# zhaoruiyang98/eftpipe

Hardware: AMD Instinct MI355X
Metric: theory P_l(k) evaluations/sec (single tracer, Nk=512, l=0,2,4) (higher is better)
Workload: dtype f64

## Files before the change

### eftpipe_amd/csrc/eftb_kernels.hpp

```cpp
#pragma once
#include <hip/hip_runtime.h>
#include <stdint.h>

namespace eftb {

constexpr int NS = 80;
constexpr int NPOW = 257;
constexpr int NHALF = 128;
constexpr int NCH = 129;

constexpr int NROW = 24;

typedef double v4d __attribute__((ext_vector_type(4)));
typedef double v2d __attribute__((ext_vector_type(2)));

__device__ __forceinline__ void xcd_decode(int ntile, int& tile, int& group) {
    const int flat = blockIdx.x, ng = gridDim.x / ntile;
    if ((ng & 7) == 0) {
        const int slot = flat >> 3;
        tile = slot % ntile;
        group = (flat & 7) + 8 * (slot / ntile);
    } else {
        tile = flat % ntile;
        group = flat / ntile;
    }
}

template <bool LO>
__device__ __forceinline__ void prep_rows_body(int Nkin, int ntail, int nxtail, int KP1, int KP2, int KP3, int Bmax,
                                                        const double* __restrict__ Pin, const double* __restrict__ lnkin,
                                                        const double* __restrict__ lnxtail, const double* __restrict__ lnxxtail,
                                                        const double* __restrict__ wq2, double* __restrict__ A1, double* __restrict__ A2,
                                                        double* __restrict__ A2T, double* __restrict__ A3, int* __restrict__ status,
                                                        int ntail_lo, int nxtail_lo) {
    extern __shared__ double sm[];
    double* pin = sm;
    const int w = blockIdx.x, tid = threadIdx.x;
    bool bad = false;
    for (int j = tid; j < Nkin; j += blockDim.x) {
        const double v = Pin[(size_t)w * Nkin + j];
        pin[j] = v;
        bad = bad || !(fabs(v) <= 1.79769313486231570815e308) || (j >= Nkin - 2 && !(v > 0.0));
        if (LO) bad = bad || (j < 2 && !(v > 0.0));
    }
    if (bad && status) atomicMax(status, w + 1);
    __syncthreads();
    const double dln = lnkin[Nkin - 1] - lnkin[Nkin - 2];
    const double dlo = LO ? lnkin[1] - lnkin[0] : 0.0;
    if (A1) {
        const double slope = (log(pin[Nkin - 1]) - log(pin[Nkin - 2])) / dln;
        const double amp = pin[Nkin - 1] * exp(-slope * lnkin[Nkin - 1]);
        double slo = 0.0, alo = 0.0;
        if (LO && ntail_lo) {
            slo = (log(pin[1]) - log(pin[0])) / dlo;
            alo = pin[0] * exp(-slo * lnkin[0]);
        }
        const int nhi = ntail - (LO ? ntail_lo : 0);
        for (int j = tid; j < KP1; j += blockDim.x) A1[(size_t)w * KP1 + j] = j < Nkin ? pin[j] : 0.0;
        for (int j = tid; j < KP2; j += blockDim.x) {
            double v = j < Nkin ? pin[j] : (j < Nkin + ntail ? amp * exp(slope * lnxtail[j - Nkin]) : 0.0);
            if (LO && j >= Nkin + nhi && j < Nkin + ntail) v = alo * exp(slo * lnxtail[j - Nkin]);
            A2[(size_t)w * KP2 + j] = v;
            A2T[(size_t)j * Bmax + w] = v;
        }
    }
    if (A3) {
        const double q1 = pin[Nkin - 1] * wq2[1], q0 = pin[Nkin - 2] * wq2[0];
        const double slope = (log(q1) - log(q0)) / dln;
        const double amp = q1 * exp(-slope * lnkin[Nkin - 1]);
        double slo = 0.0, alo = 0.0;
        if (LO && nxtail_lo) {
            const double p0 = pin[0] * wq2[2], p1 = pin[1] * wq2[3];
            slo = (log(p1) - log(p0)) / dlo;
            alo = p0 * exp(-slo * lnkin[0]);
        }
        const int nhi = nxtail - (LO ? nxtail_lo : 0);
        for (int j = tid; j < KP3; j += blockDim.x) {
            double v = j < Nkin ? pin[j] : (j < Nkin + nxtail ? amp * exp(slope * lnxxtail[j - Nkin]) : 0.0);
            if (LO && j >= Nkin + nhi && j < Nkin + nxtail) v = alo * exp(slo * lnxxtail[j - Nkin]);
            A3[(size_t)w * KP3 + j] = v;
        }
    }
}

#define PREP_ROWS_PARAMS int Nkin, int ntail, int nxtail, int KP1, int KP2, int KP3, int Bmax, const double* __restrict__ Pin, \
    const double* __restrict__ lnkin, const double* __restrict__ lnxtail, const double* __restrict__ lnxxtail, const double* __restrict__ wq2, \
    double* __restrict__ A1, double* __restrict__ A2, double* __restrict__ A2T, double* __restrict__ A3, int* __restrict__ status
#define PREP_ROWS_ARGS Nkin, ntail, nxtail, KP1, KP2, KP3, Bmax, Pin, lnkin, lnxtail, lnxxtail, wq2, A1, A2, A2T, A3, status

__global__ __launch_bounds__(256) void prep_rows_kernel(PREP_ROWS_PARAMS) {
    prep_rows_body<false>(PREP_ROWS_ARGS, 0, 0);
}

__global__ __launch_bounds__(256) void prep_rows_lo_kernel(PREP_ROWS_PARAMS, int ntail_lo, int nxtail_lo) {
    prep_rows_body<true>(PREP_ROWS_ARGS, ntail_lo, nxtail_lo);
}

__device__ __forceinline__ void qf_body(int w, int nq, const double* __restrict__ fgrow, const double* __restrict__ Qpoly, double* __restrict__ Q) {
    const int tid = threadIdx.x;
    const double f = fgrow[w];
    for (int idx = tid; idx < 2 * nq; idx += blockDim.x) {
        const int a = idx / nq, rest = idx % nq;
        const double* c = Qpoly + ((size_t)(1 - a) * nq + rest) * 15;
        double cv[15];
#pragma unroll
        for (int p = 0; p < 15; ++p) cv[p] = c[p];
        const double f2 = f * f;
        double ev = cv[14], od = cv[13];
#pragma unroll
        for (int p = 12; p >= 0; p -= 2) {
            ev = fma(ev, f2, cv[p]);
            if (p >= 1) od = fma(od, f2, cv[p - 1]);
        }
        Q[(size_t)w * 2 * nq + idx] = fma(od, f, ev);
    }
}

__global__ __launch_bounds__(256) void prep_rows_qf_kernel(int B, PREP_ROWS_PARAMS, int nq, const double* __restrict__ fgrow,
                                                           const double* __restrict__ Qpoly, double* __restrict__ Q) {
    if ((int)blockIdx.x >= B) {
        qf_body(blockIdx.x - B, nq, fgrow, Qpoly, Q);
        return;
    }
    prep_rows_body<false>(PREP_ROWS_ARGS, 0, 0);
}

__global__ __launch_bounds__(256) void prep_rows_qf_lo_kernel(int B, PREP_ROWS_PARAMS, int nq, const double* __restrict__ fgrow,
                                                              const double* __restrict__ Qpoly, double* __restrict__ Q, int ntail_lo, int nxtail_lo) {
    if ((int)blockIdx.x >= B) {
        qf_body(blockIdx.x - B, nq, fgrow, Qpoly, Q);
        return;
    }
    prep_rows_body<true>(PREP_ROWS_ARGS, ntail_lo, nxtail_lo);
}
#undef PREP_ROWS_PARAMS
#undef PREP_ROWS_ARGS

constexpr int AD_T = NHALF + 2;
constexpr int AD_CH = 1;
constexpr int KSYN = 528;
constexpr int KLIN = 288;
constexpr int SYN_KPAD = 48;
constexpr int SYN_KC = 24;
static_assert(SYN_KPAD % SYN_KC == 0 && (32 * SYN_KC) % 256 == 0, "chunk must divide the padding and fill the staging threads");
constexpr int BAS22 = 8, BASC = 32;

__device__ __forceinline__ double readlane_f64(double v, int lane) {
    return __hiloint2double(__builtin_amdgcn_readlane(__double2hiint(v), lane), __builtin_amdgcn_readlane(__double2loint(v), lane));
}

template <int NC, int NW>
__global__ __launch_bounds__(64 * NW) void antidiag_kernel(int B, int Bmax, const double* __restrict__ coefT,
                                                           const double2* __restrict__ AD, double2* __restrict__ S) {
    constexpr int PB = 3, WPP = 2 * NC;
    static_assert(PB * WPP <= 64, "one wave-load must hold a block's weights");
    __shared__ double red[NW - 1][2 * NC][64];
    const int grp = blockIdx.y, jp = (grp & 1) ? NPOW - 1 - (int)blockIdx.x : (int)blockIdx.x;
    const int lane = threadIdx.x & 63, wave = threadIdx.x >> 6, w = grp * 64 + lane;
    const int wl = w < B ? w : B - 1;
    const int cnt = ((2 * NHALF + jp) >> 1) - jp + 1;
    const int per = (cnt + NW - 1) / NW, t0 = wave * per, t1 = min(cnt, t0 + per);
    const double* cr = coefT + wl;
    const double* ci = coefT + (size_t)NCH * Bmax + wl;
    double ar[NC], ai[NC];
#pragma unroll
    for (int q = 0; q < NC; ++q) ar[q] = ai[q] = 0.0;
    if (t0 < t1) {
        const double* adw = reinterpret_cast<const double*>(AD + ((size_t)jp * AD_T + t0) * NC);
        const int nw = (t1 - t0) * WPP;
        auto wload = [&](int blk) { return adw[min(blk * PB * WPP + lane, nw - 1)]; };
        double xr[PB], xi[PB], yr[PB], yi[PB];
        auto coef = [&](int t, int p) {
            const int n = jp + t, qn = n <= NHALF ? n : 2 * NHALF - n;
            xr[p] = cr[(size_t)qn * Bmax];
            xi[p] = ci[(size_t)qn * Bmax];
            yr[p] = cr[(size_t)t * Bmax];
            yi[p] = ci[(size_t)t * Bmax];
        };
        double wc = wload(0);
#pragma unroll
        for (int p = 0; p < PB; ++p) coef(min(t0 + p, t1 - 1), p);
        const int nblk = (t1 - t0 + PB - 1) / PB;
        for (int blk = 0; blk < nblk; ++blk) {
            const double wn = wload(blk + 1);
#pragma unroll
            for (int p = 0; p < PB; ++p) {
                const int t = t0 + blk * PB + p;
                const double on = t < t1 ? 1.0 : 0.0;
                const double xim = jp + t <= NHALF ? xi[p] : -xi[p], yim = -yi[p];
                const double pr = (xr[p] * yr[p] - xim * yim) * on, pi = (xr[p] * yim + xim * yr[p]) * on;
                __builtin_amdgcn_sched_barrier(0);
                coef(min(t + PB, t1 - 1), p);
                __builtin_amdgcn_sched_barrier(0);
#pragma unroll
                for (int q = 0; q < NC; ++q) {
                    const double mx = readlane_f64(wc, p * WPP + 2 * q), my = readlane_f64(wc, p * WPP + 2 * q + 1);
                    ar[q] = fma(mx, pr, fma(-my, pi, ar[q]));
                    ai[q] = fma(mx, pi, fma(my, pr, ai[q]));
                }
                __builtin_amdgcn_sched_barrier(0);
            }
            wc = wn;
        }
    }
    if (wave > 0) {
#pragma unroll
        for (int q = 0; q < NC; ++q) {
            red[wave - 1][2 * q][lane] = ar[q];
            red[wave - 1][2 * q + 1][lane] = ai[q];
        }
    }
    __syncthreads();
    if (wave == 0 && w < B) {
#pragma unroll
        for (int q = 0; q < NC; ++q) {
#pragma unroll
            for (int v = 0; v < NW - 1; ++v) {
                ar[q] += red[v][2 * q][lane];
                ai[q] += red[v][2 * q + 1][lane];
            }
            S[((size_t)w * NC + q) * NPOW + jp] = make_double2(ar[q], ai[q]);
        }
    }
}

template <int NC, int NW>
__global__ __launch_bounds__(64 * NW) void antidiag_nh_kernel(int B, int Bmax, const double* __restrict__ coefT,
                                                              const double2* __restrict__ AD, double2* __restrict__ S, int nh) {
    constexpr int PB = 3, WPP = 2 * NC;
    static_assert(PB * WPP <= 64, "one wave-load must hold a block's weights");
    __shared__ double red[NW - 1][2 * NC][64];
    const int npow = 2 * nh + 1, nch = nh + 1, adt = nh + 2;
    const int grp = blockIdx.y, jp = (grp & 1) ? npow - 1 - (int)blockIdx.x : (int)blockIdx.x;
    const int lane = threadIdx.x & 63, wave = threadIdx.x >> 6, w = grp * 64 + lane;
    const int wl = w < B ? w : B - 1;
    const int cnt = ((2 * nh + jp) >> 1) - jp + 1;
    const int per = (cnt + NW - 1) / NW, t0 = wave * per, t1 = min(cnt, t0 + per);
    const double* cr = coefT + wl;
    const double* ci = coefT + (size_t)nch * Bmax + wl;
    double ar[NC], ai[NC];
#pragma unroll
    for (int q = 0; q < NC; ++q) ar[q] = ai[q] = 0.0;
    if (t0 < t1) {
        const double* adw = reinterpret_cast<const double*>(AD + ((size_t)jp * adt + t0) * NC);
        const int nw = (t1 - t0) * WPP;
        auto wload = [&](int blk) { return adw[min(blk * PB * WPP + lane, nw - 1)]; };
        double xr[PB], xi[PB], yr[PB], yi[PB];
        auto coef = [&](int t, int p) {
            const int n = jp + t, qn = n <= nh ? n : 2 * nh - n;
            xr[p] = cr[(size_t)qn * Bmax];
            xi[p] = ci[(size_t)qn * Bmax];
            yr[p] = cr[(size_t)t * Bmax];
            yi[p] = ci[(size_t)t * Bmax];
        };
        double wc = wload(0);
#pragma unroll
        for (int p = 0; p < PB; ++p) coef(min(t0 + p, t1 - 1), p);
        const int nblk = (t1 - t0 + PB - 1) / PB;
        for (int blk = 0; blk < nblk; ++blk) {
            const double wn = wload(blk + 1);
#pragma unroll
            for (int p = 0; p < PB; ++p) {
                const int t = t0 + blk * PB + p;
                const double on = t < t1 ? 1.0 : 0.0;
                const double xim = jp + t <= nh ? xi[p] : -xi[p], yim = -yi[p];
                const double pr = (xr[p] * yr[p] - xim * yim) * on, pi = (xr[p] * yim + xim * yr[p]) * on;
                __builtin_amdgcn_sched_barrier(0);
                coef(min(t + PB, t1 - 1), p);
                __builtin_amdgcn_sched_barrier(0);
#pragma unroll
                for (int q = 0; q < NC; ++q) {
                    const double mx = readlane_f64(wc, p * WPP + 2 * q), my = readlane_f64(wc, p * WPP + 2 * q + 1);
                    ar[q] = fma(mx, pr, fma(-my, pi, ar[q]));
                    ai[q] = fma(mx, pi, fma(my, pr, ai[q]));
                }
                __builtin_amdgcn_sched_barrier(0);
            }
            wc = wn;
        }
    }
    if (wave > 0) {
#pragma unroll
        for (int q = 0; q < NC; ++q) {
            red[wave - 1][2 * q][lane] = ar[q];
            red[wave - 1][2 * q + 1][lane] = ai[q];
        }
    }
    __syncthreads();
    if (wave == 0 && w < B) {
#pragma unroll
        for (int q = 0; q < NC; ++q) {
#pragma unroll
            for (int v = 0; v < NW - 1; ++v) {
                ar[q] += red[v][2 * q][lane];
                ai[q] += red[v][2 * q + 1][lane];
            }
            S[((size_t)w * NC + q) * npow + jp] = make_double2(ar[q], ai[q]);
// ... 218 lines not shown
        for (int e = jp; e < nrows * NCH; e += 320) {
            const int row = e / NCH, mp = e % NCH, n = NHALF - mp;
            double vx, vy;
            if (cf == 0) {
                vx = vy = 0.0;
#pragma unroll
                for (int b = 0; b < 10; ++b) {
                    const double2 v = linvec[(size_t)b * NCH + n];
                    vx = fma(s_cf[row * 38 + 28 + b], v.x, vx);
                    vy = fma(s_cf[row * 38 + 28 + b], v.y, vy);
                }
            } else {
                const double2 v = linvec[(size_t)(10 + row) * NCH + n];
                vx = s_b[row] * v.x;
                vy = s_b[row] * v.y;
            }
            const double cr = c[n], ci = n == NHALF ? 0.0 : c[NCH + n];
            double* o = out + (size_t)row * KLIN;
            if (mp == 0) o[0] = cr * vx - ci * vy;
            else {
                o[2 * mp - 1] = cr * vx - ci * vy;
                o[2 * mp] = cr * vy + ci * vx;
            }
        }
    }
}

template <int NC>
__global__ __launch_bounds__(64) void build_rows_plk_nh_kernel(int Bmax, int nb, const double* __restrict__ coef, const double2* __restrict__ S,
                                                    const double2* __restrict__ mlj, const double2* __restrict__ linvec,
                                                    const double* __restrict__ bias, const double* __restrict__ fgrow,
                                                    const double* __restrict__ l11, const double* __restrict__ lct,
                                                    const double* __restrict__ l22, const double* __restrict__ l13,
                                                    const int* __restrict__ grp, const double* __restrict__ exp22,
                                                    const double* __restrict__ expc, double* __restrict__ A22, double* __restrict__ A13,
                                                    double* __restrict__ ACF, double* __restrict__ ALC, int nh) {
    constexpr int NL = 3;
    const int npow = 2 * nh + 1, nch = nh + 1, ksyn = ksyn_of(nh), klin = klin_of(nh), zstride = 64 * (int)gridDim.z;
    __shared__ double s_cf[NL * 38];
    __shared__ double s_w[NL * NC];
    __shared__ double s_b[2 * NL];
    const int w = blockIdx.x, cf = blockIdx.y, jp = blockIdx.z * 64 + threadIdx.x;
    const double* bw = bias + (size_t)w * NROW;
    const double f = fgrow[w];
    for (int e = threadIdx.x; e < NL * 38; e += 64) {
        const int l = e / 38, bq = e % 38;
        s_cf[e] = bw[9 + grp[2 * bq]] * ipow(f, grp[2 * bq + 1]) * (bq < 28 ? l22[l * 28 + bq] : l13[l * 10 + (bq - 28)]);
    }
    if (threadIdx.x < 2 * NL) {
        const int a = threadIdx.x / NL, lp = threadIdx.x % NL;
        double v = 0.0;
        if (a == 0)
            for (int r = 0; r < 3; ++r) v = fma(bw[r], l11[lp * 3 + r], v);
        else
            for (int r = 0; r < 6; ++r) v = fma(bw[3 + r], lct[lp * 6 + r], v);
        s_b[threadIdx.x] = v;
    }
    __syncthreads();
    if (threadIdx.x < NL * NC) {
        const int l = threadIdx.x / NC, q = threadIdx.x % NC;
        double v0 = 0.0, v1 = 0.0;
        if (cf == 0) {
            if (q < nb)
                for (int b = 0; b < 28; b += 2) {
                    v0 = fma(s_cf[l * 38 + b], exp22[b * BAS22 + q], v0);
                    v1 = fma(s_cf[l * 38 + b + 1], exp22[(b + 1) * BAS22 + q], v1);
                }
        } else {
            for (int b = 0; b < 28; b += 2) {
                v0 = fma(s_cf[l * 38 + b], expc[(size_t)(l * 28 + b) * BASC + l * NC + q], v0);
                v1 = fma(s_cf[l * 38 + b + 1], expc[(size_t)(l * 28 + b + 1) * BASC + l * NC + q], v1);
            }
            for (int b = 0; b < 10; b += 2) {
                v0 = fma(s_cf[l * 38 + 28 + b], expc[(size_t)(NL * 28 + l * 10 + b) * BASC + l * NC + q], v0);
                v1 = fma(s_cf[l * 38 + 29 + b], expc[(size_t)(NL * 28 + l * 10 + b + 1) * BASC + l * NC + q], v1);
            }
        }
        s_w[threadIdx.x] = v0 + v1;
    }
    __syncthreads();
    if (jp < npow) {
        double zr[NC], zi[NC];
#pragma unroll
        for (int q = 0; q < NC; ++q) {
            zr[q] = zi[q] = 0.0;
#pragma unroll
            for (int ch = 0; ch < AD_CH; ++ch) {
                const double2 v = S[(((size_t)ch * Bmax + w) * NC + q) * npow + jp];
                zr[q] += v.x;
                zi[q] += v.y;
            }
        }
        const int o0 = jp == 0 ? 0 : 2 * jp - 1;
#pragma unroll
        for (int l = 0; l < NL; ++l) {
            double cr = 0.0, ci = 0.0;
#pragma unroll
            for (int q = 0; q < NC; ++q) {
                cr = fma(s_w[l * NC + q], zr[q], cr);
                ci = fma(s_w[l * NC + q], zi[q], ci);
            }
            if (cf == 0) {
                double* o = A22 + ((size_t)w * BAS22 + l) * ksyn;
                o[o0] = cr;
                if (jp) o[o0 + 1] = ci;
            } else {
                const double2 m = mlj[l * npow + jp];
                double* o = ACF + ((size_t)w * BASC + l) * ksyn;
                o[o0] = m.x * cr - m.y * ci;
                if (jp) o[o0 + 1] = m.x * ci + m.y * cr;
            }
        }
    }
    {
        const int nrows = cf == 0 ? NL : 2 * NL;
        double* out = cf == 0 ? A13 + (size_t)w * 10 * klin : ALC + (size_t)w * 2 * NL * klin;
        const double* c = coef + (size_t)w * 2 * nch;
        for (int e = jp; e < nrows * nch; e += zstride) {
            const int row = e / nch, mp = e % nch, n = nh - mp;
            double vx, vy;
            if (cf == 0) {
                vx = vy = 0.0;
#pragma unroll
                for (int b = 0; b < 10; ++b) {
                    const double2 v = linvec[(size_t)b * nch + n];
                    vx = fma(s_cf[row * 38 + 28 + b], v.x, vx);
                    vy = fma(s_cf[row * 38 + 28 + b], v.y, vy);
                }
            } else {
                const double2 v = linvec[(size_t)(10 + row) * nch + n];
                vx = s_b[row] * v.x;
                vy = s_b[row] * v.y;
            }
            const double cr = c[n], ci = n == nh ? 0.0 : c[nch + n];
            double* o = out + (size_t)row * klin;
            if (mp == 0) o[0] = cr * vx - ci * vy;
            else {
                o[2 * mp - 1] = cr * vx - ci * vy;
                o[2 * mp] = cr * vy + ci * vx;
            }
        }
    }
}

struct SynthDesc {
    const double* A;
    const double* Tab;
    double* out;
    const double* gscale;
    const double* xscale;
    long long a_group, o_group;
    int M, rpg, K, X;
    int wg_end, wgx;
};

constexpr int SYN_MAXP = 6;
struct SynthBatch {
    SynthDesc p[SYN_MAXP];
    int n;
};

__global__ __launch_bounds__(256) void synth_kernel(SynthBatch batch) {
    int pi = 0, wg0 = 0;
#pragma unroll
    for (int q = 0; q < SYN_MAXP - 1; ++q)
        if (q + 1 < batch.n && (int)blockIdx.x >= batch.p[q].wg_end) {
            pi = q + 1;
            wg0 = batch.p[q].wg_end;
        }
    const SynthDesc& d = batch.p[pi];
    const int wg = blockIdx.x - wg0, bx = wg % d.wgx, by = wg / d.wgx;
    constexpr int LDA = SYN_KC + 2, LDB = 80, NA = 32 * SYN_KC / 256, NB = SYN_KC * 64 / 256;
    __shared__ double As[32 * LDA];
    __shared__ double Bs[SYN_KC * LDB];
    const int tid = threadIdx.x, lane = tid & 63, wave = tid >> 6, r = lane & 15, g = lane >> 4;
    const int row0 = by * 32, x0 = bx * 64;
    const int rh = wave >> 1, xh = wave & 1;
    int offa[NA];
    unsigned amask = 0;
#pragma unroll
    for (int i = 0; i < NA; ++i) {
        const int e = tid + 256 * i, rr = e / SYN_KC, kk = e % SYN_KC, row = row0 + rr, rc = row < d.M ? row : d.M - 1;
        offa[i] = (int)((long long)(rc / d.rpg) * d.a_group + (long long)(rc % d.rpg) * d.K + kk);
        amask |= (row < d.M ? 1u : 0u) << i;
    }
    const int kb = tid >> 6, xx = tid & 63;
    const bool xlive = x0 + xx < d.X;
    const double* tb0 = d.Tab + (size_t)kb * d.X + (xlive ? x0 + xx : d.X - 1);
    const size_t tstep = (size_t)4 * d.X;
    double va[NA], vb[NB];
#pragma unroll
    for (int i = 0; i < NA; ++i) va[i] = d.A[offa[i]];
#pragma unroll
    for (int i = 0; i < NB; ++i) vb[i] = tb0[i * tstep];
    v4d acc[2] = {(v4d){0.0, 0.0, 0.0, 0.0}, (v4d){0.0, 0.0, 0.0, 0.0}};
    const int xw = x0 + xh * 32, ncol = xw + 16 < d.X ? 2 : (xw < d.X ? 1 : 0);
    for (int k0 = 0; k0 < d.K; k0 += SYN_KC) {
        __syncthreads();
#pragma unroll
        for (int i = 0; i < NA; ++i) {
            const int e = tid + 256 * i;
            As[(e / SYN_KC) * LDA + e % SYN_KC] = (amask >> i) & 1u ? va[i] : 0.0;
        }
#pragma unroll
        for (int i = 0; i < NB; ++i) Bs[(kb + 4 * i) * LDB + xx] = xlive ? vb[i] : 0.0;
        __syncthreads();
        if (k0 + SYN_KC < d.K) {
            const double* an = d.A + k0 + SYN_KC;
            const double* tn = tb0 + (size_t)(k0 + SYN_KC) * d.X;
#pragma unroll
            for (int i = 0; i < NA; ++i) va[i] = an[offa[i]];
#pragma unroll
            for (int i = 0; i < NB; ++i) vb[i] = tn[i * tstep];
        }
        if (ncol == 2) {
#pragma unroll 4
            for (int t = 0; t < SYN_KC / 4; ++t) {
                const double a = As[(rh * 16 + r) * LDA + 4 * t + g];
#pragma unroll
                for (int j = 0; j < 2; ++j)
                    acc[j] = __builtin_amdgcn_mfma_f64_16x16x4f64(a, Bs[(4 * t + g) * LDB + xh * 32 + 16 * j + r], acc[j], 0, 0, 0);
            }
        } else if (ncol == 1) {
#pragma unroll 4
            for (int t = 0; t < SYN_KC / 4; ++t)
                acc[0] = __builtin_amdgcn_mfma_f64_16x16x4f64(As[(rh * 16 + r) * LDA + 4 * t + g], Bs[(4 * t + g) * LDB + xh * 32 + r], acc[0], 0, 0, 0);
        }
    }
#pragma unroll
    for (int j = 0; j < 2; ++j)
#pragma unroll
        for (int q = 0; q < 4; ++q) {
            const int row = row0 + rh * 16 + g + 4 * q, x = x0 + xh * 32 + 16 * j + r;
            if (row < d.M && x < d.X) {
                const int grp = row / d.rpg, mem = row % d.rpg;
                double v = acc[j][q];
                if (d.gscale) v *= d.gscale[(size_t)grp * d.X + x];
                if (d.xscale) v *= d.xscale[x];
                d.out[(size_t)grp * d.o_group + (size_t)mem * d.X + x] = v;
            }
        }
}

template <int NW>
__global__ __launch_bounds__(64 * NW) void gemm_direct_kernel(SynthBatch batch) {
    __shared__ double red[NW - 1][8][64];
    int pi = 0, wg0 = 0;
#pragma unroll
    for (int q = 0; q < SYN_MAXP - 1; ++q)
        if (q + 1 < batch.n && (int)blockIdx.x >= batch.p[q].wg_end) {
            pi = q + 1;
            wg0 = batch.p[q].wg_end;
        }
    const SynthDesc& d = batch.p[pi];
    const int wg = blockIdx.x - wg0, bx = wg % d.wgx, by = wg / d.wgx;
    const int lane = threadIdx.x & 63, wave = threadIdx.x >> 6, r = lane & 15, g = lane >> 4;
    const int rowa = by * 16 + r, rc = rowa < d.M ? rowa : d.M - 1;
    const double* ap = d.A + (long long)(rc / d.rpg) * d.a_group + (long long)(rc % d.rpg) * d.K + 4 * g;
    const int x = bx * 32 + 2 * r;
    const bool pairs = !(d.X & 1);
    const int x0 = x < d.X ? x : d.X - 1, x1 = x + 1 < d.X ? x + 1 : d.X - 1;
    const double* bp = d.Tab + (size_t)(4 * g) * d.X;
    v4d acc0 = (v4d){0.0, 0.0, 0.0, 0.0}, acc1 = (v4d){0.0, 0.0, 0.0, 0.0};
    const int ng = d.K / 16, per = (ng + NW - 1) / NW, u0 = wave * per, u1 = min(ng, u0 + per);
    if (pairs) {
        const double* bq = bp + (x + 1 < d.X ? x : d.X - 2);
#pragma unroll 2
        for (int u = u0; u < u1; ++u) {
            const double4 a = *reinterpret_cast<const double4*>(ap + 16 * u);
            double2 b[4];
#pragma unroll
            for (int j = 0; j < 4; ++j) b[j] = *reinterpret_cast<const double2*>(bq + (size_t)(16 * u + j) * d.X);
            acc0 = __builtin_amdgcn_mfma_f64_16x16x4f64(a.x, b[0].x, acc0, 0, 0, 0);
            acc1 = __builtin_amdgcn_mfma_f64_16x16x4f64(a.x, b[0].y, acc1, 0, 0, 0);
            acc0 = __builtin_amdgcn_mfma_f64_16x16x4f64(a.y, b[1].x, acc0, 0, 0, 0);
            acc1 = __builtin_amdgcn_mfma_f64_16x16x4f64(a.y, b[1].y, acc1, 0, 0, 0);
            acc0 = __builtin_amdgcn_mfma_f64_16x16x4f64(a.z, b[2].x, acc0, 0, 0, 0);
            acc1 = __builtin_amdgcn_mfma_f64_16x16x4f64(a.z, b[2].y, acc1, 0, 0, 0);
            acc0 = __builtin_amdgcn_mfma_f64_16x16x4f64(a.w, b[3].x, acc0, 0, 0, 0);
            acc1 = __builtin_amdgcn_mfma_f64_16x16x4f64(a.w, b[3].y, acc1, 0, 0, 0);
        }
    } else {
#pragma unroll 2
        for (int u = u0; u < u1; ++u) {
            const double4 a = *reinterpret_cast<const double4*>(ap + 16 * u);
            const double av[4] = {a.x, a.y, a.z, a.w};
#pragma unroll
            for (int j = 0; j < 4; ++j) {
                const double* br = bp + (size_t)(16 * u + j) * d.X;
                acc0 = __builtin_amdgcn_mfma_f64_16x16x4f64(av[j], br[x0], acc0, 0, 0, 0);
                acc1 = __builtin_amdgcn_mfma_f64_16x16x4f64(av[j], br[x1], acc1, 0, 0, 0);
            }
        }
    }
    if (wave > 0) {
#pragma unroll
        for (int q = 0; q < 4; ++q) {
            red[wave - 1][q][lane] = acc0[q];
            red[wave - 1][4 + q][lane] = acc1[q];
        }
    }
    __syncthreads();
    if (wave > 0) return;
#pragma unroll
    for (int v = 0; v < NW - 1; ++v)
#pragma unroll
        for (int q = 0; q < 4; ++q) {
            acc0[q] += red[v][q][lane];
            acc1[q] += red[v][4 + q][lane];
        }
#pragma unroll
    for (int q = 0; q < 4; ++q) {
        const int row = by * 16 + g + 4 * q;
        if (row < d.M && x < d.X) {
            const int grp = row / d.rpg, mem = row % d.rpg;
            double v0 = acc0[q], v1 = acc1[q];
            if (d.gscale) {
                v0 *= d.gscale[(size_t)grp * d.X + x];
                if (x + 1 < d.X) v1 *= d.gscale[(size_t)grp * d.X + x + 1];
            }
            if (d.xscale) {
                v0 *= d.xscale[x];
                if (x + 1 < d.X) v1 *= d.xscale[x + 1];
            }
            double* o = d.out + (size_t)grp * d.o_group + (size_t)mem * d.X + x;
            if (pairs) *reinterpret_cast<double2*>(o) = make_double2(v0, v1);
            else {
                o[0] = v0;
                if (x + 1 < d.X) o[1] = v1;
            }
        }
    }
}

constexpr int EXP_RPB = 8;

template <int RIN>
__device__ inline void expand_body(int bx, int grp, int bz, int Rout, int X, const double* __restrict__ basis,
                                   const double* __restrict__ comb, double* __restrict__ out) {
    const int x = bx * 64 + threadIdx.x, r0 = bz * EXP_RPB;
    if (x >= X) return;
    double v[RIN];
#pragma unroll
    for (int c = 0; c < RIN; ++c) v[c] = basis[((size_t)grp * RIN + c) * X + x];
    double acc[EXP_RPB];
#pragma unroll
    for (int i = 0; i < EXP_RPB; ++i) acc[i] = 0.0;
#pragma unroll
    for (int c = 0; c < RIN; ++c)
#pragma unroll
        for (int i = 0; i < EXP_RPB; ++i) acc[i] = fma(comb[(size_t)min(r0 + i, Rout - 1) * RIN + c], v[c], acc[i]);
#pragma unroll
    for (int i = 0; i < EXP_RPB; ++i)
        if (r0 + i < Rout) out[((size_t)grp * Rout + r0 + i) * X + x] = acc[i];
}

__global__ __launch_bounds__(64) void expand_kernel(int n22, int Nk, int B, const double* __restrict__ Y22, const double* __restrict__ exp22,
                                                    double* __restrict__ P22, int RoutC, const double* __restrict__ YCF,
                                                    const double* __restrict__ expc, double* __restrict__ CC) {
    int wg = blockIdx.x;
    if (wg < n22) {
        const int nx = (Nk + 63) / 64, nz = (28 + EXP_RPB - 1) / EXP_RPB;
        expand_body<BAS22>(wg % nx, wg / (nx * nz), (wg / nx) % nz, 28, Nk, Y22, exp22, P22);
    } else {
        wg -= n22;
        const int nx = (NS + 63) / 64, nz = (RoutC + EXP_RPB - 1) / EXP_RPB;
        expand_body<BASC>(wg % nx, wg / (nx * nz), (wg / nx) % nz, RoutC, NS, YCF, expc, CC);
    }
}

struct GemmDesc {
    const double* A; long long a_group, a_row, a_seg; int rows, rows_per_group, nseg, kseg;
    const double* B; int ldb, ncols;
    double* C; long long c_group, c_row, c_colgroup; int cols_per_group;
};

__global__ __launch_bounds__(256, 1) void gemm_rows_kernel(GemmDesc d) {
    constexpr int MT = 4, NT = 4, ROWS = 64, KC = 256, LD = KC + 2;
    extern __shared__ double sm[];
    const int tid = threadIdx.x, lane = tid & 63, wave = tid >> 6;
    const int r = lane & 15, g = lane >> 4;
    const int row0 = blockIdx.x * ROWS, col0 = blockIdx.y * 256 + wave * 64;
    v4d acc[MT][NT];
#pragma unroll
    for (int i = 0; i < MT; ++i)
#pragma unroll
        for (int j = 0; j < NT; ++j) acc[i][j] = (v4d){0.0, 0.0, 0.0, 0.0};
    const bool wave_live = col0 < d.ncols;
    for (int seg = 0; seg < d.nseg; ++seg) {
        for (int kc0 = 0; kc0 < d.kseg; kc0 += KC) {
            const int kc = min(KC, d.kseg - kc0);
            const int kcp = (kc + 3) & ~3;
            __syncthreads();
            for (int idx = tid; idx < ROWS * (kcp / 2); idx += 256) {
// ... 2883 lines not shown
```

### eftpipe_amd/csrc/eftbird.hip

```cpp
#include "../../include/eftbird.h"

#include <hip/hip_runtime.h>
#include <dlfcn.h>
#include <rccl/rccl.h>

#include <algorithm>
#include <atomic>
#include <chrono>
#include <cmath>
#include <condition_variable>
#include <mutex>
#include <thread>
#include <cstdarg>
#include <cstdio>
#include <cstdlib>
#include <cstring>
#include <functional>
#include <string>
#include <tuple>
#include <algorithm>
#include <vector>

#include "eftb_kernels.hpp"

// ... 229 lines not shown
    volatile unsigned long long* set_done = nullptr;
    unsigned long long set_word[NSETS] = {};
    unsigned long long set_cword[NSETS] = {};
    bool plk_dma = true;
    bool done_words = true;
    static constexpr int NTP = 12, NTRACE = 64;
    hipEvent_t evTrace[NTRACE][NTP] = {};
    hipEvent_t evTraceBase = nullptr;
    int trace_B[NTRACE] = {};
    unsigned long long trace_launch[NTRACE] = {};
    bool trace_on = false;
    int trace_slot = -1;
    unsigned long long trace_n = 0;
    bool sub_stats = false;
    double issue_ns = 0.0, fill_ns = 0.0, wait_ns = 0.0;
    unsigned long long issue_n = 0, inline_n = 0;
};

static void sub_stop_thread(eftb_engine* e);
static inline void sub_drain(eftb_engine* e);

struct RcclApi {
    void* handle = nullptr;
    ncclResult_t (*GetUniqueId)(ncclUniqueId*) = nullptr;
    ncclResult_t (*CommInitRank)(ncclComm_t*, int, ncclUniqueId, int) = nullptr;
    ncclResult_t (*CommDestroy)(ncclComm_t) = nullptr;
    ncclResult_t (*GroupStart)() = nullptr;
    ncclResult_t (*GroupEnd)() = nullptr;
    ncclResult_t (*Send)(const void*, size_t, ncclDataType_t, int, ncclComm_t, hipStream_t) = nullptr;
    ncclResult_t (*Recv)(void*, size_t, ncclDataType_t, int, ncclComm_t, hipStream_t) = nullptr;
    const char* (*GetErrorString)(ncclResult_t) = nullptr;
};
static RcclApi g_rccl;

static int rccl_load() {
    if (g_rccl.handle) return 0;
    void* h = dlopen("librccl.so.1", RTLD_NOW | RTLD_GLOBAL);
    if (!h) h = dlopen("librccl.so", RTLD_NOW | RTLD_GLOBAL);
    if (!h) return fail("cannot load librccl.so: %s", dlerror());
#define RSYM(field, name)                                                 \
    g_rccl.field = reinterpret_cast<decltype(g_rccl.field)>(dlsym(h, name)); \
    if (!g_rccl.field) return fail("librccl.so lacks %s", name);
    RSYM(GetUniqueId, "ncclGetUniqueId")
    RSYM(CommInitRank, "ncclCommInitRank")
    RSYM(CommDestroy, "ncclCommDestroy")
    RSYM(GroupStart, "ncclGroupStart")
    RSYM(GroupEnd, "ncclGroupEnd")
    RSYM(Send, "ncclSend")
    RSYM(Recv, "ncclRecv")
    RSYM(GetErrorString, "ncclGetErrorString")
#undef RSYM
    g_rccl.handle = h;
    return 0;
}

#define NCCLCHK(expr)                                                                            \
    do {                                                                                         \
        ncclResult_t _r = (expr);                                                                \
        if (_r != ncclSuccess) return fail("%s failed: %s", #expr, g_rccl.GetErrorString(_r));   \
    } while (0)

static inline void trace_point(eftb_engine* e, int p, hipStream_t st) {
    if (e->trace_slot >= 0) (void)hipEventRecord(e->evTrace[e->trace_slot][p], st);
}

static inline size_t kpad(int n) { return (size_t)(n + SYN_KPAD - 1) / SYN_KPAD * SYN_KPAD; }

static inline int cfg_nh(const eftb_config& c) { return c.nfft ? c.nfft / 2 : NHALF; }
static inline int cfg_npow(const eftb_config& c) { return 2 * cfg_nh(c) + 1; }
static inline int cfg_nch(const eftb_config& c) { return cfg_nh(c) + 1; }

static size_t need_table_bytes(const eftb_config& c, int id) {
    const size_t D = sizeof(double);
    const int Nn = 2 * c.NIR * c.Na;
    switch (id) {
        case EFTB_T_K: return D * c.Nk;
        case EFTB_T_S: return D * NS;
        case EFTB_T_LNKIN: return D * c.Nkin;
        case EFTB_T_SKT: return D * kpad(c.Nkin) * c.Nk;
        case EFTB_T_GCT: case EFTB_T_ECT: return D * kpad(c.Nkin + c.ntail) * 2 * cfg_nch(c);
        case EFTB_T_LNXTAIL: return D * c.ntail;
        case EFTB_T_AD: return 2 * D * (size_t)(c.nbasis + (c.with_resum ? c.nbasis13 : 0)) * cfg_npow(c) * (cfg_nh(c) + 2);
        case EFTB_T_EXP22: return D * 28 * BAS22;
        case EFTB_T_EXPC: return c.with_resum ? D * (size_t)c.Nl * 38 * BASC : 0;
        case EFTB_T_MLJ: return c.with_resum ? 2 * D * c.Nl * cfg_npow(c) : 0;
        case EFTB_T_LINVEC: return 2 * D * (size_t)(10 + (c.with_resum ? (c.with_nnlo ? 3 : 2) * c.Nl : 0)) * cfg_nch(c);
        case EFTB_T_SYNK: return D * (size_t)ksyn_of(cfg_nh(c)) * c.Nk;
        case EFTB_T_LINK: return D * (size_t)klin_of(cfg_nh(c)) * c.Nk;
        case EFTB_T_SYNS: return c.with_resum ? D * (size_t)ksyn_of(cfg_nh(c)) * NS : 0;
        case EFTB_T_LINS: return c.with_resum ? D * (size_t)klin_of(cfg_nh(c)) * NS : 0;
        case EFTB_T_L11: return D * c.Nl * 3;
        case EFTB_T_LCT: return D * c.Nl * 6;
        case EFTB_T_L22: return D * c.Nl * 28;
        case EFTB_T_L13: return D * c.Nl * 10;
        case EFTB_T_GRP: return sizeof(int32_t) * 38 * 2;
        case EFTB_T_BXT: return c.with_resum ? D * kpad(c.Nkin + c.nxtail) * 2 * NS : 0;
        case EFTB_T_TYT: return 0;
        case EFTB_T_LNXXTAIL: return c.with_resum ? D * c.nxtail : 0;
        case EFTB_T_WQLAST2: return c.with_resum ? D * (c.nxtail_lo ? 4 : 2) : 0;
        case EFTB_T_QPOLY: return c.with_resum ? D * 2 * c.Nl * c.Nl * Nn * 15 : 0;
        case EFTB_T_H: return c.with_resum ? D * c.Na * NS * c.Nk : 0;
        case EFTB_T_RSBASIS: case EFTB_T_RSBASISS: return c.with_resum ? D * RS_NB * 16 : 0;
        case EFTB_T_RSROWS: return c.with_resum ? sizeof(int32_t) * 2 * RS3_ROWS : 0;
        case EFTB_T_MU: case EFTB_T_WMU: return c.with_ap ? D * c.nmu : 0;
        case EFTB_T_LEGMU: return c.with_ap ? D * c.Nl * c.nmu : 0;
        case EFTB_T_SPBAND: return c.with_ap ? D * (size_t)(2 * SPL_HB + 1) * c.Nk : 0;
        case EFTB_T_SPCBAND: return c.with_ap ? D * (size_t)(2 * SPL_HB + 1) * c.Nk : 0;
        case EFTB_T_SPLOCAL: return c.with_ap ? D * (size_t)16 * c.Nk : 0;
        case EFTB_T_APFID: return c.with_ap ? D * 2 : 0;
        case EFTB_T_LCTN: return c.with_nnlo ? D * c.Nl * 6 : 0;
        case EFTB_T_BAO: return c.optiresum && c.with_resum ? D * (2 * NS + 4) : 0;
        case EFTB_T_GCT2: case EFTB_T_GCT2T: return c.dual_coef ? D * kpad(c.Nkin + c.ntail) * 2 * cfg_nch(c) : 0;
    }
    return 0;
}

static size_t need_buffer_elems(const eftb_config& c, int id) {
    const size_t B = c.max_batch;
    const int Nn = 2 * c.NIR * c.Na;
    switch (id) {
        case EFTB_B_PIN: return B * c.Nkin;
        case EFTB_B_F: case EFTB_B_DA: case EFTB_B_H: return B;
        case EFTB_B_P11: return B * c.Nk;
        case EFTB_B_P22: return B * 28 * c.Nk;
        case EFTB_B_P13: return B * 10 * c.Nk;
        case EFTB_B_C11: case EFTB_B_CCT: return c.with_resum ? B * c.Nl * NS : 0;
        case EFTB_B_CC: return c.with_resum ? B * c.Nl * 38 * NS : 0;
        case EFTB_B_CLOOPL: return c.with_resum ? B * c.Nl * 12 * NS : 0;
        case EFTB_B_TEMPL: return B * c.Nl * NROW * c.Nk;
        case EFTB_B_XY: return c.with_resum ? B * 2 * NS : 0;
        case EFTB_B_Q: return c.with_resum ? B * 2 * c.Nl * c.Nl * Nn : 0;
        case EFTB_B_BIAS: return B * NROW;
        case EFTB_B_PLK: return B * c.Nl * c.Nk;
        case EFTB_B_COEF: return B * 2 * cfg_nch(c);
        case EFTB_B_GROWS: return B * MARG_NG1 * NROW;
        case EFTB_B_LOGP: return B * MARG_OUT;
        case EFTB_B_CCTN: return c.with_nnlo && c.with_resum ? B * c.Nl * NS : 0;
        case EFTB_B_TEMPLN: return c.with_nnlo ? B * c.Nl * NROW * c.Nk : 0;
        case EFTB_B_BIASN: return c.with_nnlo ? B * 3 : 0;
        case EFTB_B_GROWSN: return c.with_nnlo ? B * MARG_NG1 * 3 : 0;
    }
    return 0;
}

template <typename T>
static inline const T* tb(const eftb_engine* e, int id) { return static_cast<const T*>(e->tab[id]); }

static void queue_synth(SynthBatch& sb, const double* A, long long a_group, int groups, int rpg, int K, const double* Tab, int X, double* out,
                        long long o_group, const double* gscale, const double* xscale) {
    SynthDesc& d = sb.p[sb.n];
    d.A = A; d.Tab = Tab; d.out = out; d.gscale = gscale; d.xscale = xscale;
    d.a_group = a_group; d.o_group = o_group; d.M = groups * rpg; d.rpg = rpg; d.K = K; d.X = X;
    d.wgx = (X + 63) / 64;
    d.wg_end = (sb.n ? sb.p[sb.n - 1].wg_end : 0) + d.wgx * ((d.M + 31) / 32);
    ++sb.n;
}

static void launch_synth(hipStream_t st, const SynthBatch& sb) {
    if (sb.n) hipLaunchKernelGGL(synth_kernel, dim3(sb.p[sb.n - 1].wg_end), dim3(256), 0, st, sb);
}

static int launch_gemm_direct(hipStream_t st, SynthBatch sb, int waves = 4) {
    int end = 0;
    for (int i = 0; i < sb.n; ++i) {
        SynthDesc& d = sb.p[i];
        if (d.K % 16) return fail("eftb_run: K = %d of a first-stage product is not a multiple of 16", d.K);
        d.wgx = (d.X + 31) / 32;
        end += d.wgx * ((d.M + 15) / 16);
        d.wg_end = end;
    }
    if (sb.n && waves == 2) hipLaunchKernelGGL((gemm_direct_kernel<2>), dim3(end), dim3(128), 0, st, sb);
    else if (sb.n) hipLaunchKernelGGL((gemm_direct_kernel<4>), dim3(end), dim3(256), 0, st, sb);
    return 0;
}

static int launch_antidiag_rows(eftb_engine* e, hipStream_t st, int B, int sets, const double* coef, const double* coefT, bool contracted = false) {
    const eftb_config& c = e->c;
    const int nc = c.nbasis + (c.with_resum ? c.nbasis13 : 0);
    const int nh = cfg_nh(c), npow = 2 * nh + 1;
    const dim3 grid(npow, (B + 63) / 64), rgrid(B, 2, (npow + 63) / 64);
#define AD_ARGS B, c.max_batch, coefT, tb<double2>(e, EFTB_T_AD), e->SAD
#define ROW_ARGS sets, c.max_batch, c.Nl, c.with_nnlo ? 3 : 2, c.nbasis, coef, e->SAD, tb<double2>(e, EFTB_T_MLJ), tb<double2>(e, EFTB_T_LINVEC), e->A22, e->A13, \
                 e->ACF, e->ALC
#define PLK_ARGS c.max_batch, c.nbasis, coef, e->SAD, tb<double2>(e, EFTB_T_MLJ), tb<double2>(e, EFTB_T_LINVEC), e->buf[EFTB_B_BIAS], e->buf[EFTB_B_F], \
                 tb<double>(e, EFTB_T_L11), tb<double>(e, EFTB_T_LCT), tb<double>(e, EFTB_T_L22), tb<double>(e, EFTB_T_L13), tb<int>(e, EFTB_T_GRP), \
                 tb<double>(e, EFTB_T_EXP22), tb<double>(e, EFTB_T_EXPC), e->A22, e->A13, e->ACF, e->ALC
    if (nh != NHALF) {
        if (nc != 9 && nc != 7)
            return fail("loop-matrix basis of dimension %d + %d is not instantiated (expected 7 + 2)", c.nbasis, c.with_resum ? c.nbasis13 : 0);
        if (sets & 0x10) {
            if (nc == 9 && e->ad_waves == 2) hipLaunchKernelGGL((antidiag_nh_kernel<9, 2>), grid, dim3(128), 0, st, AD_ARGS, nh);
            else if (nc == 9) hipLaunchKernelGGL((antidiag_nh_kernel<9, 4>), grid, dim3(256), 0, st, AD_ARGS, nh);
            else if (e->ad_waves == 2) hipLaunchKernelGGL((antidiag_nh_kernel<7, 2>), grid, dim3(128), 0, st, AD_ARGS, nh);
            else hipLaunchKernelGGL((antidiag_nh_kernel<7, 4>), grid, dim3(256), 0, st, AD_ARGS, nh);
        }
        if (contracted) trace_point(e, 11, st);
        if (contracted && nc == 9) hipLaunchKernelGGL((build_rows_plk_nh_kernel<9>), rgrid, dim3(64), 0, st, PLK_ARGS, nh);
        else if (nc == 9) hipLaunchKernelGGL((build_rows_nh_kernel<9>), rgrid, dim3(64), 0, st, ROW_ARGS, nh);
        else hipLaunchKernelGGL((build_rows_nh_kernel<7>), rgrid, dim3(64), 0, st, ROW_ARGS, nh);
    } else if (nc == 9) {
        if (contracted && WHATIF_SKIP(4)) {
        } else if ((sets & 0x10) && e->ad_waves == 2) hipLaunchKernelGGL((antidiag_kernel<9, 2>), grid, dim3(128), 0, st, AD_ARGS);
        else if (sets & 0x10) hipLaunchKernelGGL((antidiag_kernel<9, 4>), grid, dim3(256), 0, st, AD_ARGS);
        if (contracted) trace_point(e, 11, st);
        if (contracted && WHATIF_SKIP(8)) {
        } else if (contracted)
            hipLaunchKernelGGL((build_rows_plk_kernel<9>), rgrid, dim3(64), 0, st, PLK_ARGS);
        else
        hipLaunchKernelGGL((build_rows_kernel<9>), rgrid, dim3(64), 0, st, ROW_ARGS);
    } else if (nc == 7) {
        if ((sets & 0x10) && e->ad_waves == 2) hipLaunchKernelGGL((antidiag_kernel<7, 2>), grid, dim3(128), 0, st, AD_ARGS);
        else if (sets & 0x10) hipLaunchKernelGGL((antidiag_kernel<7, 4>), grid, dim3(256), 0, st, AD_ARGS);
        hipLaunchKernelGGL((build_rows_kernel<7>), rgrid, dim3(64), 0, st, ROW_ARGS);
    } else {
        return fail("loop-matrix basis of dimension %d + %d is not instantiated (expected 7 + 2)", c.nbasis, c.with_resum ? c.nbasis13 : 0);
    }
#undef AD_ARGS
#undef ROW_ARGS
#undef PLK_ARGS
    return 0;
}

static int launch_operator(eftb_engine* e, int id, int B, int t0 = 0, int tstride = 1, bool commit = true) {
    if (id < 0 || id >= (int)e->ops.size()) return fail("operator id %d out of range", id);
    const eftb_engine::Op& o = e->ops[id];
    if (o.nl_in != e->cur_nl || o.nx_in != e->cur_nx)
        return fail("operator %d expects templates [%d][24][%d], the block is [%d][24][%d]", id, o.nl_in, o.nx_in, e->cur_nl, e->cur_nx);
    auto launch = [&](const eftb_engine::Op& m, int r0, int nr) {
        GemmDesc g{};
        const long long bin = (long long)o.nl_in * NROW * o.nx_in, bout = (long long)o.nl_out * NROW * o.nx_out;
        g.A = e->buf[EFTB_B_TEMPL] + (size_t)t0 * bin + (size_t)r0 * o.nx_in; g.a_group = bin * tstride; g.a_row = o.nx_in;
        g.a_seg = (long long)NROW * o.nx_in;
        g.rows = ((B - t0 + tstride - 1) / tstride) * nr; g.rows_per_group = nr; g.nseg = o.nl_in; g.kseg = o.nx_in;
        g.B = m.dev; g.ldb = m.ld; g.ncols = o.nl_out * o.nx_out;
        g.C = e->Talt + (size_t)t0 * bout + (size_t)r0 * o.nx_out; g.c_group = bout * tstride; g.c_row = o.nx_out;
        g.c_colgroup = (long long)NROW * o.nx_out;
        g.cols_per_group = o.nx_out;
        if (g.ncols <= 16 * GN_MAXT)
            hipLaunchKernelGGL(gemm_narrow_kernel, dim3((g.rows + 15) / 16, 1), dim3(256), 0, (e->opstream ? e->opstream : e->stream), g, GemmZ{});
        else
            hipLaunchKernelGGL(gemm_rows_kernel, dim3((g.rows + 63) / 64, (g.ncols + 255) / 256), dim3(256), GEMM_LDS, (e->opstream ? e->opstream : e->stream), g);
    };
    if (o.st_op < 0) launch(o, 0, NROW);
    else {
        launch(o, 0, NROW - 3);
        launch(e->ops[o.st_op], NROW - 3, 3);
    }
    if (!commit) return 0;
    std::swap(e->buf[EFTB_B_TEMPL], e->Talt);
    e->cur_nl = o.nl_out;
    e->cur_nx = o.nx_out;
    return 0;
}

static int launch_pipeline_operator(eftb_engine* e, int B) {
    if (e->tracer_ops.empty()) {
        if (e->pipeline_op < 0) return fail("eftb_run: stage PROJECT needs eftb_set_pipeline_operator");
        return launch_operator(e, e->pipeline_op, B);
    }
    if (B % e->ntr) return fail("eftb_run: batch %d is not a multiple of the %d tracers per likelihood point", B, e->ntr);
    const eftb_engine::Op& o = e->ops[e->tracer_ops[0]];
    bool one_launch = e->ntr <= GN_MAXZ && o.nl_out * o.nx_out <= 16 * GN_MAXT;
    for (int t = 0; t < e->ntr; ++t) one_launch = one_launch && e->ops[e->tracer_ops[t]].st_op < 0;
    if (!one_launch) {
        for (int t = 0; t < e->ntr; ++t)
            if (int rc = launch_operator(e, e->tracer_ops[t], B, t, e->ntr, t == e->ntr - 1)) return rc;
        return 0;
    }
    if (o.nl_in != e->cur_nl || o.nx_in != e->cur_nx)
        return fail("the tracers' operators expect templates [%d][24][%d], the block is [%d][24][%d]", o.nl_in, o.nx_in, e->cur_nl, e->cur_nx);
    GemmDesc g{};
    GemmZ z{};
    const long long bin = (long long)o.nl_in * NROW * o.nx_in, bout = (long long)o.nl_out * NROW * o.nx_out;
    g.A = e->buf[EFTB_B_TEMPL]; g.a_group = bin * e->ntr; g.a_row = o.nx_in; g.a_seg = (long long)NROW * o.nx_in;
    g.rows = (B / e->ntr) * NROW; g.rows_per_group = NROW; g.nseg = o.nl_in; g.kseg = o.nx_in;
    g.B = o.dev; g.ldb = o.ld; g.ncols = o.nl_out * o.nx_out;
    g.C = e->Talt; g.c_group = bout * e->ntr; g.c_row = o.nx_out; g.c_colgroup = (long long)NROW * o.nx_out; g.cols_per_group = o.nx_out;
    for (int t = 0; t < e->ntr; ++t) z.B[t] = e->ops[e->tracer_ops[t]].dev;
    z.a_off = bin;
    z.c_off = bout;
    hipLaunchKernelGGL(gemm_narrow_kernel, dim3((g.rows + 15) / 16, 1, e->ntr), dim3(256), 0, (e->opstream ? e->opstream : e->stream), g, z);
    std::swap(e->buf[EFTB_B_TEMPL], e->Talt);
    e->cur_nl = o.nl_out;
    e->cur_nx = o.nx_out;
    return 0;
}

static int launch_pipeline_operator_plk(eftb_engine* e, int B, hipStream_t st) {
    const bool per_tracer = !e->tracer_ops.empty();
    if (per_tracer && (B % e->ntr)) return fail("eftb_run: batch %d is not a multiple of the %d tracers per likelihood point", B, e->ntr);
    const int nz = per_tracer ? e->ntr : 1;
    const eftb_engine::Op& o = e->ops[per_tracer ? e->tracer_ops[0] : e->pipeline_op];
    GemmDesc g{};
    GemmZ z{};
    const long long bin = (long long)o.nl_in * o.nx_in, bout = (long long)o.nl_out * o.nx_out;
    g.A = e->PLK0; g.a_group = bin * nz; g.a_row = 0; g.a_seg = o.nx_in;
    g.rows = B / nz; g.rows_per_group = 1; g.nseg = o.nl_in; g.kseg = o.nx_in;
    g.B = o.dev; g.ldb = o.ld; g.ncols = o.nl_out * o.nx_out;
    g.C = e->buf[EFTB_B_PLK]; g.c_group = bout * nz; g.c_row = 0; g.c_colgroup = o.nx_out; g.cols_per_group = o.nx_out;
    if (g.ncols <= 16 * GN_MAXT && nz <= GN_MAXZ) {
        for (int t = 0; t < nz; ++t) z.B[t] = e->ops[per_tracer ? e->tracer_ops[t] : e->pipeline_op].dev;
        z.a_off = bin;
        z.c_off = bout;
        hipLaunchKernelGGL(gemm_narrow_kernel, dim3((g.rows + 15) / 16, 1, nz), dim3(256), 0, st, g, z);
    } else {
        for (int t = 0; t < nz; ++t) {
            GemmDesc gt = g;
// ... 2798 lines not shown
```

Before: 1.582 million.

## Pipeline synth GEMM with multi-stage async global-to-LDS loads and XCD tile remap

Rewrites the synth GEMM kernel's K-loop as a 4-stage shared-memory ring, with each chunk of 16 filled ahead of use. When operands are 16-byte aligned and even-sized, the fill uses direct global_load_lds; otherwise it copies through registers. Waits are hand-counted with s_waitcnt instead of two __syncthreads per chunk. Tiles are remapped so consecutive block IDs spread across the 8 XCDs, and the LDS layout is XOR-swizzled to avoid bank conflicts. It uses more shared memory, which may lower occupancy, and the hand-written vmcnt counts are fragile.

Measured after the change: 1.527 million. 3.5% lower.

```diff
diff --git a/eftpipe_amd/csrc/eftb_kernels.hpp b/eftpipe_amd/csrc/eftb_kernels.hpp
--- a/eftpipe_amd/csrc/eftb_kernels.hpp
+++ b/eftpipe_amd/csrc/eftb_kernels.hpp
@@ -141,8 +141,9 @@
 constexpr int KSYN = 528;
 constexpr int KLIN = 288;
 constexpr int SYN_KPAD = 48;
-constexpr int SYN_KC = 24;
-static_assert(SYN_KPAD % SYN_KC == 0 && (32 * SYN_KC) % 256 == 0, "chunk must divide the padding and fill the staging threads");
+constexpr int SYN_KC = 16;
+constexpr int SYN_ST = 4;
+static_assert(SYN_KPAD % SYN_KC == 0, "chunk must divide the padding");
 constexpr int BAS22 = 8, BASC = 32;
 
 __device__ __forceinline__ double readlane_f64(double v, int lane) {
@@ -667,6 +668,7 @@
     long long a_group, o_group;
     int M, rpg, K, X;
     int wg_end, wgx;
+    int vec;
 };
 
 constexpr int SYN_MAXP = 6;
@@ -675,71 +677,69 @@
     int n;
 };
 
-__global__ __launch_bounds__(256) void synth_kernel(SynthBatch batch) {
-    int pi = 0, wg0 = 0;
-#pragma unroll
-    for (int q = 0; q < SYN_MAXP - 1; ++q)
-        if (q + 1 < batch.n && (int)blockIdx.x >= batch.p[q].wg_end) {
-            pi = q + 1;
-            wg0 = batch.p[q].wg_end;
-        }
-    const SynthDesc& d = batch.p[pi];
-    const int wg = blockIdx.x - wg0, bx = wg % d.wgx, by = wg / d.wgx;
-    constexpr int LDA = SYN_KC + 2, LDB = 80, NA = 32 * SYN_KC / 256, NB = SYN_KC * 64 / 256;
-    __shared__ double As[32 * LDA];
-    __shared__ double Bs[SYN_KC * LDB];
-    const int tid = threadIdx.x, lane = tid & 63, wave = tid >> 6, r = lane & 15, g = lane >> 4;
-    const int row0 = by * 32, x0 = bx * 64;
+constexpr int SYN_AST = 32 * SYN_KC, SYN_STAGE = SYN_AST + SYN_KC * 64;
+static_assert(SYN_KC == 16, "the fill shapes below are written for 4 + 8 wave instructions per stage");
+
+template <bool VEC>
+__device__ __forceinline__ void synth_fill(double* stage, int wave, int lane, const double* asrc, const double* tab, int X, int bk, int xc0, int xc1,
+                                           int k0) {
+    double* ad = stage + wave * 128;
+    double* bd = stage + SYN_AST + wave * 256;
+    if constexpr (VEC) {
+        __builtin_amdgcn_global_load_lds((const __attribute__((address_space(1))) void*)(asrc + k0), (__attribute__((address_space(3))) void*)ad, 16, 0, 0);
+#pragma unroll
+        for (int i = 0; i < 2; ++i)
+            __builtin_amdgcn_global_load_lds((const __attribute__((address_space(1))) void*)(tab + (size_t)(k0 + bk + 2 * i) * X + xc0),
+                                             (__attribute__((address_space(3))) void*)(bd + 128 * i), 16, 0, 0);
+    } else {
+        ad[2 * lane] = asrc[k0];
+        ad[2 * lane + 1] = asrc[k0 + 1];
+#pragma unroll
+        for (int i = 0; i < 2; ++i) {
+            const double* t = tab + (size_t)(k0 + bk + 2 * i) * X;
+            bd[128 * i + 2 * lane] = t[xc0];
+            bd[128 * i + 2 * lane + 1] = t[xc1];
+        }
+    }
+}
+
+template <bool VEC>
+__device__ __forceinline__ void synth_tile(const SynthDesc& d, int row0, int x0, double* sm) {
+    const int tid = threadIdx.x, lane = tid & 63, wave = __builtin_amdgcn_readfirstlane(tid >> 6), r = lane & 15, g = lane >> 4;
     const int rh = wave >> 1, xh = wave & 1;
-    int offa[NA];
-    unsigned amask = 0;
-#pragma unroll
-    for (int i = 0; i < NA; ++i) {
-        const int e = tid + 256 * i, rr = e / SYN_KC, kk = e % SYN_KC, row = row0 + rr, rc = row < d.M ? row : d.M - 1;
-        offa[i] = (int)((long long)(rc / d.rpg) * d.a_group + (long long)(rc % d.rpg) * d.K + kk);
-        amask |= (row < d.M ? 1u : 0u) << i;
-    }
-    const int kb = tid >> 6, xx = tid & 63;
-    const bool xlive = x0 + xx < d.X;
-    const double* tb0 = d.Tab + (size_t)kb * d.X + (xlive ? x0 + xx : d.X - 1);
-    const size_t tstep = (size_t)4 * d.X;
-    double va[NA], vb[NB];
-#pragma unroll
-    for (int i = 0; i < NA; ++i) va[i] = d.A[offa[i]];
-#pragma unroll
-    for (int i = 0; i < NB; ++i) vb[i] = tb0[i * tstep];
+    const int arow = min(row0 + rh * 16 + r, d.M - 1);
+    const double* asrc = d.A + (long long)(arow / d.rpg) * d.a_group + (long long)(arow % d.rpg) * d.K + 2 * ((wave & 1) * 4 + g);
+    const int bk = 4 * wave + (lane >> 5), bcol = x0 + ((2 * (lane & 31)) ^ ((lane >> 5) << 4));
+    const int xc0 = VEC ? min(bcol, d.X - 2) : min(bcol, d.X - 1), xc1 = min(bcol + 1, d.X - 1);
+    const int aoff = rh * 256 + (g >> 1) * 32 + 2 * r + (g & 1);
+    const int boff0 = SYN_AST + g * 64 + ((xh * 32 + r) ^ ((g & 1) << 4)), boff1 = boff0 ^ 16;
     v4d acc[2] = {(v4d){0.0, 0.0, 0.0, 0.0}, (v4d){0.0, 0.0, 0.0, 0.0}};
     const int xw = x0 + xh * 32, ncol = xw + 16 < d.X ? 2 : (xw < d.X ? 1 : 0);
-    for (int k0 = 0; k0 < d.K; k0 += SYN_KC) {
-        __syncthreads();
-#pragma unroll
-        for (int i = 0; i < NA; ++i) {
-            const int e = tid + 256 * i;
-            As[(e / SYN_KC) * LDA + e % SYN_KC] = (amask >> i) & 1u ? va[i] : 0.0;
-        }
-#pragma unroll
-        for (int i = 0; i < NB; ++i) Bs[(kb + 4 * i) * LDB + xx] = xlive ? vb[i] : 0.0;
-        __syncthreads();
-        if (k0 + SYN_KC < d.K) {
-            const double* an = d.A + k0 + SYN_KC;
-            const double* tn = tb0 + (size_t)(k0 + SYN_KC) * d.X;
-#pragma unroll
-            for (int i = 0; i < NA; ++i) va[i] = an[offa[i]];
-#pragma unroll
-            for (int i = 0; i < NB; ++i) vb[i] = tn[i * tstep];
-        }
+    const int nch = d.K / SYN_KC;
+#pragma unroll
+    for (int c = 0; c < SYN_ST - 1; ++c)
+        if (c < nch) synth_fill<VEC>(sm + c * SYN_STAGE, wave, lane, asrc, d.Tab, d.X, bk, xc0, xc1, c * SYN_KC);
+    for (int c = 0; c < nch; ++c) {
+        const int behind = min(SYN_ST - 2, nch - 1 - c);
+        if (behind >= 2) asm volatile("s_waitcnt vmcnt(6) lgkmcnt(0)" ::: "memory");
+        else if (behind == 1) asm volatile("s_waitcnt vmcnt(3) lgkmcnt(0)" ::: "memory");
+        else asm volatile("s_waitcnt vmcnt(0) lgkmcnt(0)" ::: "memory");
+        __builtin_amdgcn_s_barrier();
+        const int cn = c + SYN_ST - 1;
+        if (cn < nch) synth_fill<VEC>(sm + (cn % SYN_ST) * SYN_STAGE, wave, lane, asrc, d.Tab, d.X, bk, xc0, xc1, cn * SYN_KC);
+        const double* as = sm + (c % SYN_ST) * SYN_STAGE + aoff;
+        const double* bs0 = sm + (c % SYN_ST) * SYN_STAGE + boff0;
+        const double* bs1 = sm + (c % SYN_ST) * SYN_STAGE + boff1;
         if (ncol == 2) {
-#pragma unroll 4
+#pragma unroll
             for (int t = 0; t < SYN_KC / 4; ++t) {
-                const double a = As[(rh * 16 + r) * LDA + 4 * t + g];
-#pragma unroll
-                for (int j = 0; j < 2; ++j)
-                    acc[j] = __builtin_amdgcn_mfma_f64_16x16x4f64(a, Bs[(4 * t + g) * LDB + xh * 32 + 16 * j + r], acc[j], 0, 0, 0);
+                const double a = as[64 * t];
+                acc[0] = __builtin_amdgcn_mfma_f64_16x16x4f64(a, bs0[256 * t], acc[0], 0, 0, 0);
+                acc[1] = __builtin_amdgcn_mfma_f64_16x16x4f64(a, bs1[256 * t], acc[1], 0, 0, 0);
             }
         } else if (ncol == 1) {
-#pragma unroll 4
-            for (int t = 0; t < SYN_KC / 4; ++t)
-                acc[0] = __builtin_amdgcn_mfma_f64_16x16x4f64(As[(rh * 16 + r) * LDA + 4 * t + g], Bs[(4 * t + g) * LDB + xh * 32 + r], acc[0], 0, 0, 0);
+#pragma unroll
+            for (int t = 0; t < SYN_KC / 4; ++t) acc[0] = __builtin_amdgcn_mfma_f64_16x16x4f64(as[64 * t], bs0[256 * t], acc[0], 0, 0, 0);
         }
     }
 #pragma unroll
@@ -755,6 +755,23 @@
                 d.out[(size_t)grp * d.o_group + (size_t)mem * d.X + x] = v;
             }
         }
+}
+
+__global__ __launch_bounds__(256) void synth_kernel(SynthBatch batch) {
+    __shared__ __attribute__((aligned(16))) double sm[SYN_ST * SYN_STAGE];
+    int pi = 0, wg0 = 0;
+#pragma unroll
+    for (int q = 0; q < SYN_MAXP - 1; ++q)
+        if (q + 1 < batch.n && (int)blockIdx.x >= batch.p[q].wg_end) {
+            pi = q + 1;
+            wg0 = batch.p[q].wg_end;
+        }
+    const SynthDesc& d = batch.p[pi];
+    const int wg = blockIdx.x - wg0, nty = (d.M + 31) / 32, per = (d.wg_end - wg0) >> 3, tile = (wg & 7) * per + (wg >> 3);
+    if (tile >= d.wgx * nty) return;
+    const int bx = tile / nty, by = tile % nty;
+    if (d.vec) synth_tile<true>(d, by * 32, bx * 64, sm);
+    else synth_tile<false>(d, by * 32, bx * 64, sm);
 }
 
 template <int NW>
diff --git a/eftpipe_amd/csrc/eftbird.hip b/eftpipe_amd/csrc/eftbird.hip
--- a/eftpipe_amd/csrc/eftbird.hip
+++ b/eftpipe_amd/csrc/eftbird.hip
@@ -405,7 +405,8 @@
     d.A = A; d.Tab = Tab; d.out = out; d.gscale = gscale; d.xscale = xscale;
     d.a_group = a_group; d.o_group = o_group; d.M = groups * rpg; d.rpg = rpg; d.K = K; d.X = X;
     d.wgx = (X + 63) / 64;
-    d.wg_end = (sb.n ? sb.p[sb.n - 1].wg_end : 0) + d.wgx * ((d.M + 31) / 32);
+    d.wg_end = (sb.n ? sb.p[sb.n - 1].wg_end : 0) + ((d.wgx * ((d.M + 31) / 32) + 7) & ~7);
+    d.vec = !(X & 1) && !(K & 1) && !(a_group & 1) && !(reinterpret_cast<uintptr_t>(A) & 15) && !(reinterpret_cast<uintptr_t>(Tab) & 15);
     ++sb.n;
 }
 
```
